# omarezz46/BayesDLL

Hardware: AMD Instinct MI355X
Metric: SG-HMC leapfrog steps/sec & HBM GB/s on ViT-L/32 params, 1/2/4/8 MI355X (higher is better)
Workload: dtype f32

## Files before the change

### bayesdll_amd/_lib.py

```python
from __future__ import annotations

import ctypes as C
import os
import threading

import numpy as np
import torch

HERE = os.path.dirname(os.path.abspath(__file__))
LIB_PATH = os.environ.get("BDL_SGMCMC_LIB", os.path.join(HERE, "libbdl_sgmcmc.so"))

BDL_OK = 0
CSGHMC, SGHMC, SGLD, SGHMC_GRAD, SGLD_GRAD, ADAM_SGHMC, ADAM_SGHMC_GRAD = range(7)
NOISE_NONE, NOISE_BUFFER, NOISE_PHILOX = 0, 1, 2
COLLECT_NONE, COLLECT_WELFORD_INIT, COLLECT_WELFORD, COLLECT_MEAN_INIT, COLLECT_MEAN = range(5)
MIX_BARE, MIX_PIPELINED, MIX_PACED = 0, 1, 2
ATTR_HEAD, ATTR_PRIOR, ATTR_SKIP, ATTR_GUNALIGNED = 0x1, 0x2, 0x4, 0x8
FLAG_FIRST_STEP, FLAG_RECIP_DIV, FLAG_MOMENTUM, FLAG_GRAD_READY = 0x1, 0x2, 0x4, 0x8
VAR_GIVEN, VAR_RAW_MOMENTS, VAR_WELFORD = 0, 1, 2
ABI_VERSION = 8

_fp = C.c_void_p


# ... 423 lines not shown
DIVERSITY_INT_MATRICES = ("disagree", "both_wrong", "kl_unbounded")
DIVERSITY_SUM_MATRICES = ("tv_sum", "kl_sum")


def diversity_totals_dtype(voters):
    P = int(voters)
    return np.dtype([(k, np.int64) for k in ("n", "n_labelled", "n_nonfinite", "voters")]
                    + [(k, np.int64, (P, P)) for k in DIVERSITY_INT_MATRICES]
                    + [(k, np.float64, (P, P)) for k in DIVERSITY_SUM_MATRICES])


class DiversityArgs(C.Structure):
    _fields_ = [("logits", _fp), ("labels", _fp), ("totals", _fp), ("workspace", _fp),
                ("batch", C.c_int64), ("voters", C.c_int32), ("classes", C.c_int32),
                ("grid_blocks", C.c_int32), ("flags", C.c_int32)]


DIVERSITY_EXPORTS = {
    "bdl_diversity_totals_bytes": (C.c_int64, [C.c_int32]),
    "bdl_diversity_workspace_bytes": (C.c_int64, [C.c_int32, C.c_int32]),
    "bdl_diversity": (C.c_int, [C.POINTER(DiversityArgs), C.c_void_p]),
}

_lib = None
_lock = threading.Lock()


def lib():
    global _lib
    if _lib is not None:
        return _lib
    with _lock:
        if _lib is None:
            if not os.path.exists(LIB_PATH):
                raise RuntimeError(
                    f"bayesdll_amd: HIP library not found at {LIB_PATH}; build it with "
                    "`make -C bayesdll_amd/csrc` (or __graft_entry__.build()). There is no CPU "
                    "fallback for the fused SG-MCMC step.")
            h = C.CDLL(LIB_PATH)
            for name, (res, argt) in (list(EXPORTS.items()) + list(DIAG_EXPORTS.items())
                                      + list(CLIP_EXPORTS.items())
                                      + list(CHAIN_STEP_EXPORTS.items())
                                      + list(STATS_EXPORTS.items())
                                      + list(ESS_EXPORTS.items())
                                      + list(LOWP_EXPORTS.items())
                                      + list(LAYERS_EXPORTS.items())
                                      + list(PREDICT_EXPORTS.items())
                                      + list(FN_EXPORTS.items())
                                      + list(TEMPER_EXPORTS.items())
                                      + list(MIXTURE_EXPORTS.items())
                                      + list(RANK_EXPORTS.items())
                                      + list(DIVERSITY_EXPORTS.items())):
                fn = getattr(h, name)
                fn.restype = res
                fn.argtypes = argt
            if h.bdl_version() != ABI_VERSION:
                raise RuntimeError(f"bayesdll_amd: ABI version mismatch ({h.bdl_version()} != "
                                   f"{ABI_VERSION}); rebuild the library")
            _lib = h
    return _lib


def check(rc: int, what: str):
    if rc != BDL_OK:
        msg = lib().bdl_last_error().decode(errors="replace")
        raise RuntimeError(f"{what} failed (status {rc}): {msg}")
    return rc


def ptr(t):
    return None if t is None else C.c_void_p(t.data_ptr())


def current_stream_handle(device=None):
    return C.c_void_p(torch.cuda.current_stream(device).cuda_stream)
# ... 9 lines not shown
```

### bayesdll_amd/csrc/bdl_api.hip

```cpp
#include <algorithm>
#include "bdl_chain_common.hpp"
#include "bdl_measure.h"

#include <mutex>
#include <vector>

namespace bdl {
namespace {

thread_local std::string g_last_error;

int g_blocks_per_cu = 2;
int g_unroll = 1;
int g_grid_stride = 1;

int device_cu_count() {
  static int cached[64] = {0};
  int dev = 0;
  if (hipGetDevice(&dev) != hipSuccess || dev < 0 || dev >= 64) return 256;
  if (cached[dev] == 0) {
    int cus = 0;
    if (hipDeviceGetAttribute(&cus, hipDeviceAttributeMultiprocessorCount, dev) != hipSuccess ||
        cus <= 0)
      cus = 256;
// ... 407 lines not shown
    return fail(BDL_ERR_RUNS, std::string(what) + ": run table exceeds 64 KiB of LDS (4096 runs, "
                "2730 with grad_base; merge parameter groups)");
  if (!s->grad && !s->grad_base)
    return fail(BDL_ERR_NULL, std::string(what) + ": grad or grad_base is required");
  if (misaligned(s->grad, 15))
    return fail(BDL_ERR_ALIGN, std::string(what) + ": grad not 16-B aligned");
  if (misaligned(s->grad_base, 7))
    return fail(BDL_ERR_ALIGN, std::string(what) + ": grad_base not 8-B aligned");
  if (s->chain_groups &&
      (s->chain_groups > 0xFFFFFFFFull ||
       (uint64_t)((s->n + 3) / 4) + s->philox_offset > 0xFFFFFFFFull))
    return fail(BDL_ERR_ARG, std::string(what) + ": stacked chains need every float4 group "
                "index below 2^32 (chain_groups, n / 4 + philox_offset)");
  if (s->noise_mode == BDL_NOISE_PHILOX)
    return check_philox_range(what, s->n, s->philox_offset, s->chain, s->chain_groups);
  return BDL_OK;
}

std::mutex g_captured_mu;
std::vector<const void*> g_captured_funcs;
thread_local hipGraphExec_t g_redirect_exec = nullptr;
thread_local hipGraphNode_t g_redirect_node = nullptr;

int launch_step(const bdl_step_args* s, const float* clip, hipStream_t stream, bool bare = false) {
  if (!s) return fail(BDL_ERR_NULL, "bdl_sgmcmc_step: null args");
  if (s->n < 0) return fail(BDL_ERR_ARG, "bdl_sgmcmc_step: n < 0");
  if (s->method < BDL_CSGHMC || s->method > BDL_SGLD_GRAD)
    return fail(BDL_ERR_ARG, "bdl_sgmcmc_step: unknown method");
  if (s->noise_mode < BDL_NOISE_NONE || s->noise_mode > BDL_NOISE_PHILOX)
    return fail(BDL_ERR_ARG, "bdl_sgmcmc_step: unknown noise mode");
  if (s->collect < BDL_COLLECT_NONE || s->collect > BDL_COLLECT_MEAN)
    return fail(BDL_ERR_ARG, "bdl_sgmcmc_step: unknown collect mode");
  if (s->n == 0) return BDL_OK;
  const bool grad_only = s->method == BDL_SGHMC_GRAD || s->method == BDL_SGLD_GRAD;
  const bool needs_mom = s->method == BDL_CSGHMC || s->method == BDL_SGHMC ||
                         s->method == BDL_SGHMC_GRAD ||
                         (s->method == BDL_SGLD && (s->flags & BDL_FLAG_MOMENTUM));
  const bool needs_prior = s->method != BDL_CSGHMC;
  if (!s->theta) return fail(BDL_ERR_NULL, "bdl_sgmcmc_step: theta is required");
  if (const int rc = check_runs_and_grad(s, "bdl_sgmcmc_step")) return rc;
  if (needs_mom && !s->mom) return fail(BDL_ERR_NULL, "bdl_sgmcmc_step: mom is required");
  if (needs_prior && !s->prior_mean)
    return fail(BDL_ERR_NULL, "bdl_sgmcmc_step: prior_mean is required for sghmc/sgld");
  if (s->noise_mode == BDL_NOISE_BUFFER && !s->noise)
    return fail(BDL_ERR_NULL, "bdl_sgmcmc_step: noise buffer is required");
  if (s->collect != BDL_COLLECT_NONE && !s->mom1)
    return fail(BDL_ERR_NULL, "bdl_sgmcmc_step: mom1 is required to collect");
// ... 10 lines not shown
  if (!k) return fail(BDL_ERR_ARG, "bdl_sgmcmc_step: unsupported method/noise/collect combination");

  const int64_t ngroups = (s->n + 3) / 4;
  const int64_t per_iter = (int64_t)kBlock * unroll;
  const int64_t cap = (int64_t)device_cu_count() * g_blocks_per_cu;
  int64_t iters = (ngroups + per_iter - 1) / per_iter;
  int64_t grid = capped_grid(iters, cap);
  int64_t iters_per_block = (iters + grid - 1) / grid;
  grid = (iters + iters_per_block - 1) / iters_per_block;

  KArgs a;
  a.theta = s->theta;
  a.grad = s->grad;
  a.mom = s->mom;
  a.prior_mean = s->prior_mean;
  a.noise = s->noise;
  a.mom1 = s->mom1;
  a.mom2 = s->mom2;
  a.runs = s->runs;
  a.gbase = s->grad_base;
  a.nruns = s->nruns;
  a.flags = s->flags;
  a.n = s->n;
  a.groups_per_block = g_grid_stride ? 0 : iters_per_block * per_iter;
  a.lr0 = s->lr[0];
  a.lr1 = s->lr[1];
  a.ns0 = s->noise_scale[0];
  a.ns1 = s->noise_scale[1];
  a.one_minus_alpha = s->one_minus_alpha;
  a.prior_sig = s->prior_sig;
  a.sigma2 = s->sigma2;
  a.n_data = s->n_data;
  a.mu = s->mu;
  a.ca = s->collect_a;
  a.cb = s->collect_b;
  a.seed = s->seed;
  a.chain = s->chain;
  a.step = s->step;
  a.clip = clip;
  a.nonfinite = s->nonfinite;
  a.goff = s->philox_offset;
  a.cgroups = (uint32_t)s->chain_groups;
  a.inv_s2 = recip_or(s->inv_sigma2, s->sigma2);
  a.inv_nd = recip_or(s->inv_n_data, s->n_data);
  a.inv_ca = recip_or(s->inv_collect_a, s->collect_a);
  a.inv_cb = recip_or(s->inv_collect_b, s->collect_b);

  if (g_redirect_exec) {
    hipGraphNodeType nt = hipGraphNodeTypeEmpty;
    hipKernelNodeParams cur{};
    if (hipGraphNodeGetType(g_redirect_node, &nt) != hipSuccess || nt != hipGraphNodeTypeKernel ||
        hipGraphKernelNodeGetParams(g_redirect_node, &cur) != hipSuccess ||
        cur.func != (void*)k) {
      (void)hipGetLastError();
      return fail(BDL_ERR_ARG, "bdl_sgmcmc_step: the redirect node is not this step's kernel");
    }
    void* kp[] = {&a};
    hipKernelNodeParams p{};
    p.func = (void*)k;
    p.gridDim = dim3((unsigned)grid);
    p.blockDim = dim3(kBlock);
    p.sharedMemBytes = (unsigned)run_lds_bytes(s);
    p.kernelParams = kp;
    const hipError_t err = hipGraphExecKernelNodeSetParams(g_redirect_exec, g_redirect_node, &p);
    if (err != hipSuccess) {
      (void)hipGetLastError();
      g_last_error = std::string("bdl_sgmcmc_step: graph node update failed: ") +
                     hipGetErrorString(err);
      return BDL_ERR_LAUNCH;
    }
// ... 191 lines not shown
  const KArgs* ka = (const KArgs*)p.kernelParams[0];
  const int64_t v[10] = {(int64_t)(uintptr_t)ka->theta, (int64_t)(uintptr_t)ka->grad,
                         (int64_t)(uintptr_t)ka->mom,   (int64_t)(uintptr_t)ka->runs,
                         (int64_t)(uintptr_t)ka->gbase, (int64_t)ka->nruns,
                         ka->n,                          (int64_t)ka->flags,
                         (int64_t)(uintptr_t)ka->mom1,  (int64_t)(uintptr_t)ka->mom2};
  for (int i = 0; i < 10; ++i) out[i] = v[i];
  return BDL_OK;
}

int bdl_graph_redirect(void* graph_exec, void* node) {
  if (graph_exec && !node) return fail(BDL_ERR_NULL, "bdl_graph_redirect: null node");
  g_redirect_exec = (hipGraphExec_t)graph_exec;
  g_redirect_node = graph_exec ? (hipGraphNode_t)node : nullptr;
  return BDL_OK;
}

const char* bdl_last_error(void) { return g_last_error.c_str(); }

int bdl_set_launch_config(int32_t blocks_per_cu, int32_t unroll, int32_t grid_stride) {
  const int prev = (g_grid_stride << 24) | (g_blocks_per_cu << 8) | g_unroll;
  g_blocks_per_cu = blocks_per_cu > 0 ? blocks_per_cu : 2;
  g_unroll = (unroll == 1 || unroll == 2 || unroll == 4) ? unroll : 1;
  g_grid_stride = grid_stride > 0 ? 1 : 0;
  return prev;
}

int bdl_build_runs(const bdl_segment* segs, int32_t nseg, int64_t n, bdl_run* out, int32_t max_runs) {
  if (!out || (nseg > 0 && !segs)) return fail(BDL_ERR_NULL, "bdl_build_runs: null pointer");
  if (n < 0 || nseg < 0 || max_runs < 1) return fail(BDL_ERR_ARG, "bdl_build_runs: bad sizes");
  int nr = 0;
  int64_t pos = 0;
  auto push = [&](int64_t end, uint32_t attr) -> bool {
    if (end <= pos) return true;
    if (nr > 0 && out[nr - 1].attr == attr) {
      out[nr - 1].end = end;
    } else {
      if (nr >= max_runs) return false;
      out[nr].end = end;
      out[nr].attr = attr;
      out[nr].pad = 0;
      ++nr;
    }
    pos = end;
    return true;
  };
  for (int i = 0; i < nseg; ++i) {
    const bdl_segment& s = segs[i];
// ... 297 lines not shown
```

### bayesdll_amd/csrc/bdl_kernels.hpp

```cpp
#pragma once
#include <hip/hip_runtime.h>

#include <stdint.h>
#include <stdio.h>
#include <string.h>

#include <algorithm>
#include <string>

#include "bdl_sgmcmc.h"

namespace bdl {

constexpr int kBlock = 256;

__device__ __forceinline__ uint4 philox4x32_10(uint4 c, uint32_t k0, uint32_t k1) {
#ifdef BDL_PHILOX_KEYS_PER_CALL
  asm volatile("" : "+s"(k0), "+s"(k1));
#endif
#if defined(BDL_PHILOX_ROUND_KEYS_PER_CALL) && !defined(BDL_PHILOX_KEYS_PER_CALL)
  asm volatile("" : "+s"(k0), "+s"(k1));
#endif
#pragma unroll
  for (int i = 0; i < 10; ++i) {
    const uint64_t p0 = (uint64_t)0xD2511F53u * c.x;
    const uint64_t p1 = (uint64_t)0xCD9E8D57u * c.z;
    const uint32_t hi0 = (uint32_t)(p0 >> 32), lo0 = (uint32_t)p0;
    const uint32_t hi1 = (uint32_t)(p1 >> 32), lo1 = (uint32_t)p1;
#ifdef BDL_PHILOX_TWO_XORS
    c = make_uint4(hi1 ^ c.y ^ k0, lo1, hi0 ^ c.w ^ k1, lo0);
#else
    c = make_uint4(__builtin_amdgcn_bitop3_b32(hi1, c.y, k0, 0x96), lo1,
                   __builtin_amdgcn_bitop3_b32(hi0, c.w, k1, 0x96), lo0);
// ... 703 lines not shown

template <int METHOD, int NOISE, int COLLECT, bool RECIP, int UNROLL>
__device__ __forceinline__ void step_variant(const KArgs& a) {
  if constexpr (COLLECT != BDL_COLLECT_NONE || !(METHOD == BDL_SGLD || METHOD == BDL_SGHMC)) {
    step_body<METHOD, NOISE, COLLECT, RECIP, UNROLL, kVarRuntime>(a);
  } else {
    if (a.flags & BDL_FLAG_GRAD_READY)
      step_body<METHOD, NOISE, COLLECT, RECIP, UNROLL, kVarGradReady>(a);
    else if (METHOD == BDL_SGLD && a.clip != nullptr)
      step_body<METHOD, NOISE, COLLECT, RECIP, UNROLL, kVarClip>(a);
    else
      step_body<METHOD, NOISE, COLLECT, RECIP, UNROLL, 0>(a);
  }
}

template <int METHOD, int NOISE, int COLLECT, int UNROLL>
__global__ __launch_bounds__(kBlock) void bdl_step_kernel(const KArgs a) {
  if (a.flags & BDL_FLAG_RECIP_DIV)
    step_variant<METHOD, NOISE, COLLECT, true, UNROLL>(a);
  else
    step_variant<METHOD, NOISE, COLLECT, false, UNROLL>(a);
}

struct AdamConst {
  bool sgd_mom, sgd_mom_read, has_m2, grad_is_mom;
  float inv_s2, inv_nd, inv_temp, inv_bc1, inv_bc2, inv_ca, inv_cb;
};

template <int NOISE, bool RECIP, bool PRIOR, bool GRADONLY, class A>
__device__ __forceinline__ void adam_core(const A& a, const AdamConst& c, float eta, float& th,
                                          float& g, float& vm, float& m, float& v, float& buf,
                                          float th0, float eps) {
  const float gs = sdiv<RECIP>(g, a.temp, c.inv_temp);
  float gU = gs;
  if constexpr (PRIOR) {
    const float d = th - th0;
    const float e = sdiv<RECIP>(d, a.sigma2, c.inv_s2);
    gU = gs + sdiv<RECIP>(e, a.n_data, c.inv_nd);
  }
  m = m * a.b1 + gU * a.omb1;
  v = v * a.b2 + (gU * gU) * a.omb2;
  const float mh = sdiv<RECIP>(m, a.bc1, c.inv_bc1);
  const float vh = sdiv<RECIP>(v, a.bc2, c.inv_bc2);
  const float den = sqrtf(vh) + a.aeps;
  const float pg = mh / den;
  const float pt = 1.0f / den;
// ... 491 lines not shown
    case BDL_COLLECT_MEAN_INIT:
      return pick_unroll<METHOD, NOISE, BDL_COLLECT_MEAN_INIT>(unroll);
    case BDL_COLLECT_MEAN:
      return pick_unroll<METHOD, NOISE, BDL_COLLECT_MEAN>(unroll);
  }
  return nullptr;
}

template <int METHOD>
StepKernel pick_noise(int noise, int collect, int unroll) {
  switch (noise) {
    case BDL_NOISE_NONE:
      return pick_collect<METHOD, BDL_NOISE_NONE>(collect, unroll);
    case BDL_NOISE_BUFFER:
      return pick_collect<METHOD, BDL_NOISE_BUFFER>(collect, unroll);
    case BDL_NOISE_PHILOX:
      return pick_collect<METHOD, BDL_NOISE_PHILOX>(collect, unroll);
  }
  return nullptr;
}

StepKernel pick_step_csghmc(int noise, int collect, int unroll);
StepKernel pick_step_csghmc_bare(int collect, int unroll);
StepKernel pick_step_sghmc(int method, int noise, int collect, int unroll);
StepKernel pick_step_sgld(int method, int noise, int collect, int unroll);
StepKernel pick_adam(int noise, int collect, bool grad_only, int unroll);

}
```

### bayesdll_amd/flat.py

```python
from __future__ import annotations

import contextlib
import ctypes as C

import numpy as np
import torch

from . import _lib as L
from .arena import default_grad_arena


def segment_attrs(names, readout_name, bias, requires_grad):
    attrs = []
    for nm, rg in zip(names, requires_grad):
        a = 0
        if readout_name is not None and readout_name in nm:
            a |= L.ATTR_HEAD
        if not ("bias" in nm and bias == "uninformative"):
            a |= L.ATTR_PRIOR
        if not rg:
            a |= L.ATTR_SKIP
        attrs.append(a)
    return attrs

# ... 358 lines not shown

    def bucket_state(self, bucket, ptrs, table=None):
        from types import SimpleNamespace
        start, end, idx = bucket
        nt = len(idx)
        if table is None:
            key = (start, tuple(ptrs))
            tab = self._grad_tables.get(key)
            if tab is None:
                dev = self.bucket_host_table(bucket, ptrs).pin_memory().to(self.device,
                                                                            non_blocking=True)
                tab = (dev[:2 * nt].view(nt, 2), nt, dev[2 * nt:])
                if len(self._grad_tables) >= 4 * GRAD_TABLE_CACHE:
                    self._grad_tables.pop(next(iter(self._grad_tables)))
                self._grad_tables[key] = tab
        else:
            if table.numel() != 3 * nt or table.dtype != torch.int64 or table.device != self.device:
                raise ValueError("bucket_state: table must be 3 x (bucket tensors) int64 on the device")
            tab = (table[:2 * nt].view(nt, 2), nt, table[2 * nt:])
        sl = (lambda v: None if v is None else v[start:end])
        return SimpleNamespace(theta=self.theta[start:end], grad=None, gbase=tab[2], runs=tab[0],
                               nruns=tab[1], mom=sl(self.mom), prior=sl(self.prior), noise=None,
                               n=end - start, device=self.device, nonfinite=self.nonfinite,
                               extra={k: v[start:end] for k, v in self.extra.items()}, timer=None)

    def grad_table(self):
        return (self.runs, self.nruns, self.gbase, self._untouched)

    def use_grad_table(self, t):
        self.runs, self.nruns, self.gbase, self._untouched = t

    def has_grad(self, i):
        if not self.requires_grad[i]:
            return False
        if self.grad_mode == "tensor":
            return i not in self._untouched
        return not self._touched or self._touched[i]

    def check_bound(self):
        vec, esz = (self.theta, 4) if self.shadow is None else (self.shadow, 2)
        for nm, p, o in zip(self.names, self.params, self.offsets):
            if p.data.data_ptr() != vec.data_ptr() + esz * o:
                raise RuntimeError(f"bayesdll_amd: parameter {nm!r} was re-allocated outside the "
                                   "sampler; rebuild the sampler state")

    def refresh_shadow(self):
        if self.shadow is not None:
# ... 74 lines not shown
```

### bayesdll_amd/kernels.py

```python
from __future__ import annotations

import ctypes as C
import os

import numpy as np
import torch

from . import _lib as L
from . import ess as E

DIV_MODE = os.environ.get("BDL_DIV_MODE", "recip")


def _div_flag(div_mode=None):
    return L.FLAG_RECIP_DIV if (div_mode or DIV_MODE) == "recip" else 0


def _inv(s):
    s = float(s)
    return 1.0 / s if s != 0.0 else 0.0


def _step_args(state, method, *, lrs, noise_scale, noise_mode, one_minus_alpha=1.0,
               prior_sig=0.0, sigma2=1.0, n_data=1.0, mu=0.0, first_step=False,
# ... 97 lines not shown
        gbs = [nb / (t * 1e-3) / 1e9 for t, (_, _, nb) in zip(ms, self.recs)]
        out = {"launches": self.count, "timed": len(ms), "avg_ms": sum(ms) / len(ms),
               "gbs": sum(gbs) / len(gbs)}
        if reset:
            self.count, self.recs = 0, []
        return out


def launch_kind(collect):
    if collect in (L.COLLECT_WELFORD, L.COLLECT_MEAN):
        return "collect"
    if collect in (L.COLLECT_WELFORD_INIT, L.COLLECT_MEAN_INIT):
        return "init"
    return "step"


def _launch(state, fn, a, adam=None, written=None):
    kind = launch_kind(a.collect)
    pend = getattr(state, "_tune_pending", None)
    if pend and written is not None and int(a.n) == int(state.n) and kind in pend and \
            not (a.flags & L.FLAG_FIRST_STEP) and \
            not torch.cuda.is_current_stream_capturing():
        _tune_kind(state, fn, kind, written)
    _use_geometry(state, kind)
    t = getattr(state, "timer", None)
    e0 = t.begin() if t is not None else None
    fn()
    if e0 is not None:
        t.end(e0, alg_bytes_per_elem(a, adam) * int(a.n))


def _written(state, method, *, grad_only, mom, extra=(), mom1=None, mom2=None):
    if grad_only:
        if getattr(state, "grad", None) is None:
            return None
        out = [state.grad]
    else:
        out = [state.theta]
    out += [t for t in (mom,) + tuple(extra) + (mom1, mom2) if t is not None]
    return out


LOWP_UNROLL = 4


def lowp_args(state, method, *, blocks=0, unroll=LOWP_UNROLL, **kw):
    if method not in (L.CSGHMC, L.SGHMC, L.SGLD):
# ... 35 lines not shown
    L.require_hip(theta, "theta")
    L.check(L.lib().bdl_lowp_shadow(theta.data_ptr(), shadow.data_ptr(), None, 0,
                                    int(theta.numel()), L.current_stream_handle(theta.device)),
            "bdl_lowp_shadow")


def sgmcmc_step(state, method, **kw):
    if getattr(state, "shadow", None) is not None:
        return lowp_step(state, method, **kw)
    a = _step_args(state, method, **kw)
    mb = kw.get("mom_buf")
    wr = _written(state, method, grad_only=method in (L.SGHMC_GRAD, L.SGLD_GRAD),
                  mom=state.mom if mb is None else mb,
                  mom1=kw.get("mom1") if kw.get("collect", L.COLLECT_NONE) else None,
                  mom2=kw.get("mom2") if kw.get("collect", L.COLLECT_NONE) else None)
    _launch(state, lambda: L.check(L.lib().bdl_sgmcmc_step(a, L.current_stream_handle(state.device)),
                                   "bdl_sgmcmc_step"), a, written=wr)


def sgmcmc_step_bare(state, **kw):
    a = _step_args(state, L.CSGHMC, **kw)
    L.check(L.lib().bdl_sgmcmc_step_bare(a, L.current_stream_handle(state.device)),
            "bdl_sgmcmc_step_bare")


def adam_step(state, method, *, adam_m, adam_v, sgd_buf=None, beta1, beta2, eps, t,
              momentum_decay, nd, temperature=1.0, grad_is_mom=False, lrs, noise_mode,
              sigma2, n_data, mu=0.0, first_step=False, momentum=False, collect=L.COLLECT_NONE,
              mom1=None, mom2=None, collect_a=1.0, collect_b=1.0, seed=0, chain=0, step=0,
              div_mode=None, noise=None, philox_offset=0):
    a = _step_args(state, method, lrs=lrs, noise_scale=(0.0, 0.0), noise_mode=noise_mode,
                   one_minus_alpha=1 - momentum_decay, sigma2=sigma2, n_data=n_data, mu=mu,
                   first_step=first_step, momentum=momentum, collect=collect, mom1=mom1,
                   mom2=mom2, collect_a=collect_a, collect_b=collect_b, seed=seed, chain=chain,
                   step=step, div_mode=div_mode, noise=noise, philox_offset=philox_offset)
    ad = L.AdamArgs()
    ad.adam_m = adam_m.data_ptr()
    ad.adam_v = adam_v.data_ptr()
    ad.sgd_buf = None if sgd_buf is None else sgd_buf.data_ptr()
    ad.beta1, ad.one_minus_beta1 = float(beta1), 1 - float(beta1)
    ad.beta2, ad.one_minus_beta2 = float(beta2), 1 - float(beta2)
    bc1, bc2 = 1 - float(beta1) ** int(t), 1 - float(beta2) ** int(t)
    ad.bias_corr1, ad.bias_corr2 = bc1, bc2
    ad.eps = float(eps)
    ad.two_alpha = 2 * float(momentum_decay)
    ad.nd = float(nd)
# ... 1250 lines not shown
        t.end(e0, alg_bytes_per_elem(a) * int(a.n1) * K_)


def philox_normal(n, seed, chain, step, device="cuda"):
    out = torch.empty(n, dtype=torch.float32, device=device)
    L.check(L.lib().bdl_philox_normal(out.data_ptr(), int(n), int(seed), int(chain), int(step),
                                      L.current_stream_handle(out.device)), "bdl_philox_normal")
    return out


_ACTIVE = [None]
LIBRARY_DEFAULT = (2, 1, 1)


def set_launch_config(blocks_per_cu=0, unroll=0, grid_stride=0):
    _ACTIVE[0] = (int(blocks_per_cu), int(unroll), int(grid_stride))
    return L.lib().bdl_set_launch_config(int(blocks_per_cu), int(unroll), int(grid_stride))


def restore_launch_config(packed):
    return set_launch_config((packed >> 8) & 0xFFFF, packed & 0xFF, (packed >> 24) & 0xFF)


def _use_geometry(state, kind="step"):
    cfg = getattr(state, {"collect": "collect_cfg", "init": "init_cfg"}.get(kind, "launch_cfg"),
                  None)
    if cfg is None:
        cfg = getattr(state, "launch_cfg", None)
    if cfg is not None and cfg != _ACTIVE[0]:
        set_launch_config(*cfg)


AUTOTUNE_CANDIDATES = ((2, 1, 1), (1, 4, 1), (3, 1, 1), (2, 4, 1), (1, 2, 1), (2, 2, 1))
AUTOTUNE_BY_METHOD = {
    "csghmc": AUTOTUNE_CANDIDATES + ((3, 4, 1), (1, 1, 1)),
    "sgld": AUTOTUNE_CANDIDATES + ((3, 4, 1), (4, 4, 1), (1, 1, 1)),
    "adam": AUTOTUNE_CANDIDATES + ((1, 1, 1), (4, 4, 1)),
}
_TUNED = {}
_TUNED_COLLECT = {}
COLLECT_EXTRA = ((1, 1, 1),)


ADAM_EXTRA = ("adam_m", "adam_v", "sgd_buf")


def _scratch_launcher(n, dev, method):
    return _scratch_launchers(n, dev, method)[0]


def _scratch_launchers(n, dev, method):
    from .flat import FlatState, moment_pair
    st = FlatState.from_segments([("w", (int(n),))], None, device=dev,
                                 need_prior=method != "csghmc",
                                 extra=ADAM_EXTRA if method == "adam" else ())
    st.theta.zero_()
    if method == "csghmc":
        kw = dict(lrs=(1e-4, 1e-4), noise_scale=(0.0, 0.0), noise_mode=L.NOISE_NONE,
# ... 95 lines not shown
def request_state_tuning(state, method):
    if os.environ.get("BDL_AUTOTUNE", "1") == "0" or int(state.n) < TUNE_ON_STATE_MIN:
        return
    state._tune_pending = {"step", "collect", "init"}
    state._tune_method = method
    state.tuned = {}


def _tune_kind(state, fn, kind, written):
    state._tune_pending.discard(kind)
    cands = tuple(AUTOTUNE_BY_METHOD.get(state._tune_method, AUTOTUNE_CANDIDATES))
    if kind != "step":
        cands += tuple(c for c in COLLECT_EXTRA if c not in cands)
    nf = getattr(state, "nonfinite", None)
    written = list(written) + ([nf] if nf is not None else [])
    need = sum(w.numel() * w.element_size() for w in written)
    free, _ = torch.cuda.mem_get_info(state.device)
    if need > TUNE_SNAPSHOT_FRACTION * free:
        state.tuned[kind] = {"skipped": f"snapshot {need >> 20} MiB > "
                                        f"{TUNE_SNAPSHOT_FRACTION:g} x free {free >> 20} MiB"}
        return
    best, times = tune_on_state(fn, written, cands, state.device)
    setattr(state, {"collect": "collect_cfg", "init": "init_cfg"}.get(kind, "launch_cfg"), best)
    state.tuned[kind] = {"best": best, "ms": {f"{c[0]}wg/cu x{c[1]}": round(t, 4)
                                              for c, t in times.items()}}


def tune_on_state(launch, written, candidates, device, reps=4):
    import numpy as np
    saved = [w.clone() for w in written]
    prev = _ACTIVE[0]
    ts = torch.cuda.current_stream(device)

    def measure(cfgs, k):
        out = {}
        for cfg in cfgs:
            set_launch_config(*cfg)
            launch()
            ev = [(torch.cuda.Event(enable_timing=True), torch.cuda.Event(enable_timing=True))
                  for _ in range(k)]
            for e0, e1 in ev:
                e0.record(ts)
                launch()
                e1.record(ts)
            torch.cuda.synchronize(device)
            out[cfg] = float(np.median([x.elapsed_time(y) for x, y in ev]))
            for w, s in zip(written, saved):
                w.copy_(s)
# ... 48 lines not shown
```

Measured before the change: 926.3.

## Add dynamic atomic work-claiming order for cSGHMC sweep and autotune it

Adds a third sweep order for the cSGHMC step. Workgroups claim fixed-size chunks through a per-stream device atomic counter pair instead of static spans or grid-stride, which is meant to even out tail imbalance across workgroups. The dynamic variants are added to the cSGHMC autotune candidates, so they are used only when the tuner picks them. Bucketed sub-states fall back to grid-stride. A drift probe kernel that records per-workgroup timestamps is also added for diagnostics. The cost is an atomic per chunk, an extra syncthreads, and a host-side claim-ring lookup plus stream-capture check on every launch.

```diff
diff --git a/bayesdll_amd/_lib.py b/bayesdll_amd/_lib.py
--- a/bayesdll_amd/_lib.py
+++ b/bayesdll_amd/_lib.py
@@ -469,6 +469,18 @@
     "bdl_diversity": (C.c_int, [C.POINTER(DiversityArgs), C.c_void_p]),
 }
 
+ORDER_SPANS, ORDER_GRID_STRIDE, ORDER_DYNAMIC = 0, 1, 2
+CLAIM_GROUPS, CLAIM_SLOTS, CLAIM_SLOTS_PER_STREAM = 2048, 16, 4
+DRIFT_EVERY, DRIFT_SAMPLES = 16, 64
+DRIFT_WORDS = 4 + 2 * DRIFT_SAMPLES
+
+ORDER_EXPORTS = {
+    "bdl_order_last": (C.c_int, [C.POINTER(C.c_int32)]),
+    "bdl_order_counters": (C.c_int, [C.c_int32, C.POINTER(C.c_uint32)]),
+    "bdl_sweep_drift": (C.c_int, [C.POINTER(StepArgs), C.c_int32, C.c_void_p, C.c_int64,
+                                  C.POINTER(C.c_int32), C.c_void_p]),
+}
+
 _lib = None
 _lock = threading.Lock()
 
@@ -497,7 +509,8 @@
                                       + list(TEMPER_EXPORTS.items())
                                       + list(MIXTURE_EXPORTS.items())
                                       + list(RANK_EXPORTS.items())
-                                      + list(DIVERSITY_EXPORTS.items())):
+                                      + list(DIVERSITY_EXPORTS.items())
+                                      + list(ORDER_EXPORTS.items())):
                 fn = getattr(h, name)
                 fn.restype = res
                 fn.argtypes = argt
diff --git a/bayesdll_amd/csrc/bdl_api.hip b/bayesdll_amd/csrc/bdl_api.hip
--- a/bayesdll_amd/csrc/bdl_api.hip
+++ b/bayesdll_amd/csrc/bdl_api.hip
@@ -1,5 +1,6 @@
 #include <algorithm>
 #include "bdl_chain_common.hpp"
+#include "bdl_claim_ring.hpp"
 #include "bdl_measure.h"
 
 #include <mutex>
@@ -453,7 +454,54 @@
 thread_local hipGraphExec_t g_redirect_exec = nullptr;
 thread_local hipGraphNode_t g_redirect_node = nullptr;
 
-int launch_step(const bdl_step_args* s, const float* clip, hipStream_t stream, bool bare = false) {
+constexpr int kClaimStride = 32;
+struct DeviceClaims {
+  uint32_t* base = nullptr;
+  ClaimRing ring{};
+};
+std::mutex g_claim_mu;
+DeviceClaims g_claims[64];
+thread_local int g_last_order = -1, g_last_slot = -1;
+
+uint32_t* claim_pair(hipStream_t stream, int* slot) {
+  bool capturing = false;
+  if (stream) {
+    hipStreamCaptureStatus cs = hipStreamCaptureStatusNone;
+    capturing = hipStreamIsCapturing(stream, &cs) != hipSuccess || cs != hipStreamCaptureStatusNone;
+    (void)hipGetLastError();
+  }
+  const bool redirect = g_redirect_exec != nullptr;
+  int dev = 0;
+  if (capturing || redirect || hipGetDevice(&dev) != hipSuccess || dev < 0 || dev >= 64)
+    return nullptr;
+  std::lock_guard<std::mutex> lk(g_claim_mu);
+  DeviceClaims& d = g_claims[dev];
+  if (!d.base) {
+    const size_t bytes = (size_t)BDL_CLAIM_SLOTS * kClaimStride * sizeof(uint32_t);
+    uint32_t* p = nullptr;
+    if (hipMalloc((void**)&p, bytes) != hipSuccess || hipMemset(p, 0, bytes) != hipSuccess ||
+        hipDeviceSynchronize() != hipSuccess) {
+      (void)hipGetLastError();
+      if (p) (void)hipFree(p);
+      return nullptr;
+    }
+    d.base = p;
+  }
+  const int sl = claim_ring_next(d.ring, (uintptr_t)stream, capturing, redirect);
+  if (sl < 0) return nullptr;
+  *slot = sl;
+  return d.base + (size_t)sl * kClaimStride;
+}
+
+struct DriftReq {
+  int order;
+  uint64_t* records;
+  int64_t record_bytes;
+  int32_t* grid;
+};
+
+int launch_step(const bdl_step_args* s, const float* clip, hipStream_t stream, bool bare = false,
+                const DriftReq* drift = nullptr) {
   if (!s) return fail(BDL_ERR_NULL, "bdl_sgmcmc_step: null args");
   if (s->n < 0) return fail(BDL_ERR_ARG, "bdl_sgmcmc_step: n < 0");
   if (s->method < BDL_CSGHMC || s->method > BDL_SGLD_GRAD)
@@ -510,7 +558,8 @@
   a.nruns = s->nruns;
   a.flags = s->flags;
   a.n = s->n;
-  a.groups_per_block = g_grid_stride ? 0 : iters_per_block * per_iter;
+  const int order = drift ? drift->order : g_grid_stride;
+  a.groups_per_block = order ? 0 : iters_per_block * per_iter;
   a.lr0 = s->lr[0];
   a.lr1 = s->lr[1];
   a.ns0 = s->noise_scale[0];
@@ -534,6 +583,31 @@
   a.inv_ca = recip_or(s->inv_collect_a, s->collect_a);
   a.inv_cb = recip_or(s->inv_collect_b, s->collect_b);
 
+  int slot = -1;
+  uint32_t* pair = nullptr;
+  if (order == 2 && s->method == BDL_CSGHMC &&
+      run_lds_bytes(s) + 16 <= (size_t)kMaxRuns * sizeof(bdl_run))
+    pair = claim_pair(stream, &slot);
+  g_last_order = pair ? 2 : (order ? 1 : 0);
+  g_last_slot = slot;
+  const int32_t citers = (int32_t)(BDL_CLAIM_GROUPS / per_iter);
+  if (pair) grid = capped_grid((iters + citers - 1) / citers, cap);
+  if (drift) {
+    if (order == 2 && !pair)
+      return fail(BDL_ERR_ARG, "bdl_sweep_drift: no counter pair for the dynamic order here");
+    if (drift->record_bytes < grid * (int64_t)(BDL_DRIFT_WORDS * sizeof(uint64_t)))
+      return fail(BDL_ERR_ARG, "bdl_sweep_drift: records too small for the launch's workgroups");
+    *drift->grid = (int32_t)grid;
+    hipLaunchKernelGGL(pick_drift(unroll, pair != nullptr), dim3((unsigned)grid), dim3(kBlock),
+                       run_lds_bytes(s), stream, a, pair, citers, drift->records);
+    return launched("bdl_sweep_drift");
+  }
+  if (pair) {
+    hipLaunchKernelGGL(pick_step_csghmc_dyn(s->noise_mode, s->collect, unroll, bare),
+                       dim3((unsigned)grid), dim3(kBlock), run_lds_bytes(s), stream, a, pair, citers);
+    return launched("bdl_sgmcmc_step");
+  }
+
   if (g_redirect_exec) {
     hipGraphNodeType nt = hipGraphNodeTypeEmpty;
     hipKernelNodeParams cur{};
@@ -771,8 +845,54 @@
   const int prev = (g_grid_stride << 24) | (g_blocks_per_cu << 8) | g_unroll;
   g_blocks_per_cu = blocks_per_cu > 0 ? blocks_per_cu : 2;
   g_unroll = (unroll == 1 || unroll == 2 || unroll == 4) ? unroll : 1;
-  g_grid_stride = grid_stride > 0 ? 1 : 0;
+  g_grid_stride = grid_stride == 2 ? 2 : (grid_stride > 0 ? 1 : 0);
   return prev;
+}
+
+int bdl_order_last(int32_t* slot) {
+  if (slot) *slot = g_last_slot;
+  return g_last_order;
+}
+
+int bdl_order_counters(int32_t device, uint32_t* out) {
+  if (!out) return fail(BDL_ERR_NULL, "bdl_order_counters: null out");
+  if (device < 0 || device >= 64) return fail(BDL_ERR_ARG, "bdl_order_counters: bad device");
+  std::fill(out, out + 2 * BDL_CLAIM_SLOTS, 0u);
+  std::lock_guard<std::mutex> lk(g_claim_mu);
+  const uint32_t* base = g_claims[device].base;
+  if (!base) return BDL_OK;
+  int cur = 0;
+  uint32_t host[BDL_CLAIM_SLOTS * kClaimStride];
+  if (hipGetDevice(&cur) != hipSuccess || hipSetDevice(device) != hipSuccess) {
+    (void)hipGetLastError();
+    return fail(BDL_ERR_LAUNCH, "bdl_order_counters: cannot select the device");
+  }
+  const bool ok = hipDeviceSynchronize() == hipSuccess &&
+                  hipMemcpy(host, base, sizeof(host), hipMemcpyDeviceToHost) == hipSuccess;
+  (void)hipSetDevice(cur);
+  if (!ok) {
+    (void)hipGetLastError();
+    return fail(BDL_ERR_LAUNCH, "bdl_order_counters: reading the counters failed");
+  }
+  for (int i = 0; i < BDL_CLAIM_SLOTS; ++i) {
+    out[2 * i] = host[i * kClaimStride];
+    out[2 * i + 1] = host[i * kClaimStride + 1];
+  }
+  return BDL_OK;
+}
+
+int bdl_sweep_drift(const bdl_step_args* s, int32_t order, uint64_t* records, int64_t record_bytes,
+                    int32_t* grid, void* stream) {
+  if (const int rc = no_redirect("bdl_sweep_drift")) return rc;
+  if (!s || !records || !grid) return fail(BDL_ERR_NULL, "bdl_sweep_drift: null argument");
+  if (s->method != BDL_CSGHMC || s->noise_mode != BDL_NOISE_NONE || s->collect != BDL_COLLECT_NONE)
+    return fail(BDL_ERR_ARG, "bdl_sweep_drift: the probe runs the cSGHMC explore sweep only "
+                "(no noise, no collect)");
+  if (order < 0 || order > 2) return fail(BDL_ERR_ARG, "bdl_sweep_drift: order must be 0, 1 or 2");
+  if (misaligned(records, 7)) return fail(BDL_ERR_ALIGN, "bdl_sweep_drift: records not 8-B aligned");
+  if (s->n == 0) return fail(BDL_ERR_ARG, "bdl_sweep_drift: n == 0");
+  const DriftReq req{order, records, record_bytes, grid};
+  return launch_step(s, nullptr, (hipStream_t)stream, false, &req);
 }
 
 int bdl_build_runs(const bdl_segment* segs, int32_t nseg, int64_t n, bdl_run* out, int32_t max_runs) {
diff --git a/bayesdll_amd/csrc/bdl_claim_ring.hpp b/bayesdll_amd/csrc/bdl_claim_ring.hpp
--- /dev/null
+++ b/bayesdll_amd/csrc/bdl_claim_ring.hpp
@@ -0,0 +1,29 @@
+#pragma once
+#include <stdint.h>
+
+#include "bdl_order.h"
+
+namespace bdl {
+
+struct ClaimRing {
+  uintptr_t owner[BDL_CLAIM_SLOTS];
+  bool bound[BDL_CLAIM_SLOTS];
+  int cursor;
+};
+
+inline int claim_ring_next(ClaimRing& ring, uintptr_t stream, bool capturing, bool redirect) {
+  if (capturing || redirect) return -1;
+  int owned = 0;
+  for (int i = 0; i < BDL_CLAIM_SLOTS; ++i) owned += ring.bound[i] && ring.owner[i] == stream;
+  for (int k = 0; k < BDL_CLAIM_SLOTS; ++k) {
+    const int s = (ring.cursor + k) % BDL_CLAIM_SLOTS;
+    if (ring.bound[s] ? ring.owner[s] != stream : owned >= BDL_CLAIM_SLOTS_PER_STREAM) continue;
+    ring.bound[s] = true;
+    ring.owner[s] = stream;
+    ring.cursor = (s + 1) % BDL_CLAIM_SLOTS;
+    return s;
+  }
+  return -1;
+}
+
+}
diff --git a/bayesdll_amd/csrc/bdl_kernels.hpp b/bayesdll_amd/csrc/bdl_kernels.hpp
--- a/bayesdll_amd/csrc/bdl_kernels.hpp
+++ b/bayesdll_amd/csrc/bdl_kernels.hpp
@@ -9,6 +9,7 @@
 #include <string>
 
 #include "bdl_sgmcmc.h"
+#include "bdl_order.h"
 
 namespace bdl {
 
@@ -758,6 +759,155 @@
     step_variant<METHOD, NOISE, COLLECT, false, UNROLL>(a);
 }
 
+struct NoProbe {
+  __device__ __forceinline__ void begin() {}
+  __device__ __forceinline__ void tick(int64_t) {}
+  __device__ __forceinline__ void end() {}
+};
+
+struct DriftProbe {
+  uint64_t* __restrict__ rec;
+  uint32_t it;
+  __device__ __forceinline__ void begin() {
+    if (threadIdx.x == 0) rec[0] = wall_clock64();
+  }
+  __device__ __forceinline__ void tick(int64_t iter) {
+    if (it % BDL_DRIFT_EVERY == 0) {
+      const uint32_t s = it / BDL_DRIFT_EVERY;
+      if (s < BDL_DRIFT_SAMPLES && threadIdx.x == 0) {
+        rec[4 + 2 * s] = wall_clock64();
+        rec[5 + 2 * s] = (uint64_t)iter;
+      }
+    }
+    ++it;
+  }
+  __device__ __forceinline__ void end() {
+    __threadfence();
+    __syncthreads();
+    if (threadIdx.x == 0) {
+      rec[1] = wall_clock64();
+      rec[2] = min((it + BDL_DRIFT_EVERY - 1) / BDL_DRIFT_EVERY, (uint32_t)BDL_DRIFT_SAMPLES);
+      rec[3] = it;
+    }
+  }
+};
+
+template <int METHOD, int NOISE, int COLLECT, bool RECIP, int UNROLL, bool DYN, class PROBE>
+__device__ __forceinline__ void csg_sweep(const KArgs& a, uint32_t* __restrict__ claim,
+                                          int32_t citers, PROBE probe) {
+  static_assert(is_csghmc_sweep<METHOD>(), "the dynamic order exists for the cSGHMC sweeps");
+  __shared__ uint32_t s_claim[2];
+  const StepConst c = make_step_const<METHOD, COLLECT, kVarRuntime>(a);
+  const int64_t ngroups = (a.n + 3) >> 2;
+  const int64_t nfull = a.n >> 2;
+  constexpr int64_t kIter = (int64_t)kBlock * UNROLL;
+  const int64_t cgroups = (int64_t)citers * kIter;
+  int64_t g0, g1, gstep;
+  if constexpr (DYN) {
+    g0 = (int64_t)blockIdx.x * cgroups;
+    g1 = min(g0 + cgroups, ngroups);
+    gstep = kIter;
+  } else if (a.groups_per_block > 0) {
+    g0 = (int64_t)blockIdx.x * a.groups_per_block;
+    g1 = min(g0 + a.groups_per_block, ngroups);
+    gstep = kIter;
+  } else {
+    g0 = (int64_t)blockIdx.x * kIter;
+    g1 = ngroups;
+    gstep = (int64_t)gridDim.x * kIter;
+  }
+  stage_runs(a);
+  probe.begin();
+  uint32_t bad = 0, nxt = 0;
+  int r = -1, par = 0;
+  while (g0 < g1) {
+    if constexpr (DYN) {
+      if (threadIdx.x == 0) nxt = gridDim.x + atomicAdd(claim, 1u);
+    }
+    if (r < 0) r = find_run_lds(a.nruns, g0 * 4);
+    if constexpr (COLLECT != BDL_COLLECT_NONE && !csg_collect_per_run<COLLECT, UNROLL>()) {
+      for (int64_t gb = g0; gb < g1; gb += gstep) {
+        while (r < a.nruns - 1 && run_end(r) <= gb * 4) ++r;
+        const int64_t gend = min(gb + kIter, g1);
+        const uint32_t attr = run_attr(r);
+        const bool full = gend == gb + kIter && gend <= nfull;
+        if (full && run_end(r) >= gend * 4 && !(attr & kNoFastPath))
+          chunk_fast_dispatch<METHOD, NOISE, COLLECT, RECIP, UNROLL>(a, c, gb, attr,
+                                                                      run_grad(a, r), bad);
+        else if (full && multi_run_ok(a.nruns, r, gend * 4))
+          chunk_multi<METHOD, NOISE, COLLECT, RECIP, UNROLL>(a, c, gb, r, bad);
+        else
+          chunk_slow<METHOD, NOISE, COLLECT, RECIP, UNROLL>(a, c, gb, gend, r, bad);
+        probe.tick(gb / kIter);
+      }
+    } else {
+      for (int64_t gb = g0; gb < g1;) {
+        while (r < a.nruns - 1 && run_end(r) <= gb * 4) ++r;
+        const uint32_t attr = run_attr(r);
+        const int64_t lim = min(min(run_end(r) >> 2, nfull), g1);
+        if (!(attr & kNoFastPath) && gb + kIter <= lim) {
+          const bool head = (attr & BDL_ATTR_HEAD) != 0;
+          const float eta = head ? a.lr1 : a.lr0, ns = head ? a.ns1 : a.ns0;
+          float* gp = run_grad(a, r);
+          do {
+            chunk_fast<METHOD, NOISE, COLLECT, RECIP, UNROLL, false, false>(a, c, gb, eta, ns, gp,
+                                                                            bad);
+            probe.tick(gb / kIter);
+            gb += gstep;
+          } while (gb + kIter <= lim);
+          continue;
+        }
+        const int64_t gend = min(gb + kIter, g1);
+        if (gend == gb + kIter && gend <= nfull && multi_run_ok(a.nruns, r, gend * 4))
+          chunk_multi<METHOD, NOISE, COLLECT, RECIP, UNROLL>(a, c, gb, r, bad);
+        else
+          chunk_slow<METHOD, NOISE, COLLECT, RECIP, UNROLL>(a, c, gb, gend, r, bad);
+        probe.tick(gb / kIter);
+        gb += gstep;
+      }
+    }
+    if constexpr (!DYN) {
+      break;
+    } else {
+      if (threadIdx.x == 0) s_claim[par] = nxt;
+      __syncthreads();
+      const uint32_t blk = s_claim[par];
+      par ^= 1;
+      g0 = (int64_t)blk * cgroups;
+      g1 = min(g0 + cgroups, ngroups);
+    }
+  }
+  report_nonfinite(a, bad);
+  probe.end();
+  if constexpr (DYN) {
+    if (threadIdx.x == 0 && atomicAdd(claim + 1, 1u) == gridDim.x - 1) {
+      __hip_atomic_store(claim, 0u, __ATOMIC_RELAXED, __HIP_MEMORY_SCOPE_AGENT);
+      __hip_atomic_store(claim + 1, 0u, __ATOMIC_RELAXED, __HIP_MEMORY_SCOPE_AGENT);
+    }
+  }
+}
+
+template <int METHOD, int NOISE, int COLLECT, int UNROLL>
+__global__ __launch_bounds__(kBlock) void bdl_step_dyn_kernel(const KArgs a, uint32_t* claim,
+                                                              int32_t citers) {
+  if (a.flags & BDL_FLAG_RECIP_DIV)
+    csg_sweep<METHOD, NOISE, COLLECT, true, UNROLL, true, NoProbe>(a, claim, citers, NoProbe{});
+  else
+    csg_sweep<METHOD, NOISE, COLLECT, false, UNROLL, true, NoProbe>(a, claim, citers, NoProbe{});
+}
+
+template <int UNROLL, bool DYN>
+__global__ __launch_bounds__(kBlock) void bdl_drift_kernel(const KArgs a, uint32_t* claim,
+                                                           int32_t citers, uint64_t* rec) {
+  DriftProbe p{rec + (size_t)blockIdx.x * BDL_DRIFT_WORDS, 0};
+  if (a.flags & BDL_FLAG_RECIP_DIV)
+    csg_sweep<BDL_CSGHMC, BDL_NOISE_NONE, BDL_COLLECT_NONE, true, UNROLL, DYN, DriftProbe>(
+        a, claim, citers, p);
+  else
+    csg_sweep<BDL_CSGHMC, BDL_NOISE_NONE, BDL_COLLECT_NONE, false, UNROLL, DYN, DriftProbe>(
+        a, claim, citers, p);
+}
+
 struct AdamConst {
   bool sgd_mom, sgd_mom_read, has_m2, grad_is_mom;
   float inv_s2, inv_nd, inv_temp, inv_bc1, inv_bc2, inv_ca, inv_cb;
@@ -1295,6 +1445,10 @@
 
 StepKernel pick_step_csghmc(int noise, int collect, int unroll);
 StepKernel pick_step_csghmc_bare(int collect, int unroll);
+using DynKernel = void (*)(const KArgs, uint32_t*, int32_t);
+using DriftKernel = void (*)(const KArgs, uint32_t*, int32_t, uint64_t*);
+DynKernel pick_step_csghmc_dyn(int noise, int collect, int unroll, bool bare);
+DriftKernel pick_drift(int unroll, bool dyn);
 StepKernel pick_step_sghmc(int method, int noise, int collect, int unroll);
 StepKernel pick_step_sgld(int method, int noise, int collect, int unroll);
 StepKernel pick_adam(int noise, int collect, bool grad_only, int unroll);
diff --git a/bayesdll_amd/csrc/bdl_step_csghmc_dyn.hip b/bayesdll_amd/csrc/bdl_step_csghmc_dyn.hip
--- /dev/null
+++ b/bayesdll_amd/csrc/bdl_step_csghmc_dyn.hip
@@ -0,0 +1,61 @@
+#include "bdl_kernels.hpp"
+
+namespace bdl {
+namespace {
+
+template <int METHOD, int NOISE, int COLLECT>
+DynKernel dyn_unroll(int unroll) {
+  switch (unroll) {
+    case 1:
+      return bdl_step_dyn_kernel<METHOD, NOISE, COLLECT, 1>;
+    case 4:
+      return bdl_step_dyn_kernel<METHOD, NOISE, COLLECT, 4>;
+    default:
+      return bdl_step_dyn_kernel<METHOD, NOISE, COLLECT, 2>;
+  }
+}
+
+template <int METHOD, int NOISE>
+DynKernel dyn_collect(int collect, int unroll) {
+  switch (collect) {
+    case BDL_COLLECT_NONE:
+      return dyn_unroll<METHOD, NOISE, BDL_COLLECT_NONE>(unroll);
+    case BDL_COLLECT_WELFORD_INIT:
+      return dyn_unroll<METHOD, NOISE, BDL_COLLECT_WELFORD_INIT>(unroll);
+    case BDL_COLLECT_WELFORD:
+      return dyn_unroll<METHOD, NOISE, BDL_COLLECT_WELFORD>(unroll);
+    case BDL_COLLECT_MEAN_INIT:
+      return dyn_unroll<METHOD, NOISE, BDL_COLLECT_MEAN_INIT>(unroll);
+    case BDL_COLLECT_MEAN:
+      return dyn_unroll<METHOD, NOISE, BDL_COLLECT_MEAN>(unroll);
+  }
+  return nullptr;
+}
+
+}
+
+DynKernel pick_step_csghmc_dyn(int noise, int collect, int unroll, bool bare) {
+  if (bare) return dyn_collect<kMethodBare, BDL_NOISE_NONE>(collect, unroll);
+  switch (noise) {
+    case BDL_NOISE_NONE:
+      return dyn_collect<BDL_CSGHMC, BDL_NOISE_NONE>(collect, unroll);
+    case BDL_NOISE_BUFFER:
+      return dyn_collect<BDL_CSGHMC, BDL_NOISE_BUFFER>(collect, unroll);
+    case BDL_NOISE_PHILOX:
+      return dyn_collect<BDL_CSGHMC, BDL_NOISE_PHILOX>(collect, unroll);
+  }
+  return nullptr;
+}
+
+DriftKernel pick_drift(int unroll, bool dyn) {
+  switch (unroll) {
+    case 1:
+      return dyn ? bdl_drift_kernel<1, true> : bdl_drift_kernel<1, false>;
+    case 4:
+      return dyn ? bdl_drift_kernel<4, true> : bdl_drift_kernel<4, false>;
+    default:
+      return dyn ? bdl_drift_kernel<2, true> : bdl_drift_kernel<2, false>;
+  }
+}
+
+}
diff --git a/bayesdll_amd/flat.py b/bayesdll_amd/flat.py
--- a/bayesdll_amd/flat.py
+++ b/bayesdll_amd/flat.py
@@ -404,7 +404,8 @@
         return SimpleNamespace(theta=self.theta[start:end], grad=None, gbase=tab[2], runs=tab[0],
                                nruns=tab[1], mom=sl(self.mom), prior=sl(self.prior), noise=None,
                                n=end - start, device=self.device, nonfinite=self.nonfinite,
-                               extra={k: v[start:end] for k, v in self.extra.items()}, timer=None)
+                               extra={k: v[start:end] for k, v in self.extra.items()}, timer=None,
+                               bucket=True)
 
     def grad_table(self):
         return (self.runs, self.nruns, self.gbase, self._untouched)
diff --git a/bayesdll_amd/kernels.py b/bayesdll_amd/kernels.py
--- a/bayesdll_amd/kernels.py
+++ b/bayesdll_amd/kernels.py
@@ -143,7 +143,7 @@
             not (a.flags & L.FLAG_FIRST_STEP) and \
             not torch.cuda.is_current_stream_capturing():
         _tune_kind(state, fn, kind, written)
-    _use_geometry(state, kind)
+    _use_geometry(state, kind, sub=getattr(state, "bucket", False))
     t = getattr(state, "timer", None)
     e0 = t.begin() if t is not None else None
     fn()
@@ -225,6 +225,57 @@
     a = _step_args(state, L.CSGHMC, **kw)
     L.check(L.lib().bdl_sgmcmc_step_bare(a, L.current_stream_handle(state.device)),
             "bdl_sgmcmc_step_bare")
+
+
+def last_order():
+    slot = C.c_int32(-1)
+    return int(L.lib().bdl_order_last(C.byref(slot))), int(slot.value)
+
+
+def order_counters(device=None):
+    dev = _device(device)
+    out = (C.c_uint32 * (2 * L.CLAIM_SLOTS))()
+    L.check(L.lib().bdl_order_counters(int(dev.index or 0), out), "bdl_order_counters")
+    return np.ctypeslib.as_array(out).reshape(L.CLAIM_SLOTS, 2).copy()
+
+
+def sweep_drift(state, order, **kw):
+    a = _step_args(state, L.CSGHMC, noise_mode=L.NOISE_NONE, **kw)
+    cap = 16 * 1024
+    rec = torch.zeros(cap, L.DRIFT_WORDS, dtype=torch.int64, device=state.device)
+    grid = C.c_int32(0)
+    L.check(L.lib().bdl_sweep_drift(a, int(order), rec.data_ptr(),
+                                    rec.numel() * rec.element_size(), C.byref(grid),
+                                    L.current_stream_handle(state.device)), "bdl_sweep_drift")
+    torch.cuda.synchronize(state.device)
+    return rec[:grid.value].cpu()
+
+
+def drift_summary(rec, fractions=(0.125, 0.25, 0.375, 0.5, 0.625, 0.75, 0.875)):
+    rec = rec.numpy().astype(np.int64)
+    t0, t1, ns = rec[:, 0], rec[:, 1], rec[:, 2]
+    start, end = int(t0.min()), int(t1.max())
+    span = end - start
+    grid = rec.shape[0]
+    out = {"workgroups": int(grid), "span_ticks": int(span),
+           "iterations": int(rec[:, 3].sum()),
+           "iterations_min_max": [int(rec[:, 3].min()), int(rec[:, 3].max())],
+           "tail_loss": float(1.0 - (t1 - t0).sum() / (grid * span)),
+           "ramp_loss": float((t0 - start).sum() / (grid * span)),
+           "end_loss": float((end - t1).sum() / (grid * span)),
+           "truncated": bool((rec[:, 3] > L.DRIFT_EVERY * L.DRIFT_SAMPLES).any()),
+           "spread": []}
+    ts, it = rec[:, 4::2], rec[:, 5::2]
+    valid = np.arange(L.DRIFT_SAMPLES)[None, :] < ns[:, None]
+    for f in fractions:
+        T = start + f * span
+        seen = valid & (ts <= T)
+        have = seen.any(axis=1)
+        last = np.where(seen, it, -1).max(axis=1)[have]
+        sp = int(last.max() - last.min()) if last.size else 0
+        out["spread"].append({"at": f, "iterations": sp, "rows": round(sp / grid, 2),
+                              "workgroups_sampled": int(have.sum())})
+    return out
 
 
 def adam_step(state, method, *, adam_m, adam_v, sgd_buf=None, beta1, beta2, eps, t,
@@ -1521,18 +1572,24 @@
     return set_launch_config((packed >> 8) & 0xFFFF, packed & 0xFF, (packed >> 24) & 0xFF)
 
 
-def _use_geometry(state, kind="step"):
+def _use_geometry(state, kind="step", sub=False):
     cfg = getattr(state, {"collect": "collect_cfg", "init": "init_cfg"}.get(kind, "launch_cfg"),
                   None)
     if cfg is None:
         cfg = getattr(state, "launch_cfg", None)
+    if sub:
+        act = cfg or _ACTIVE[0]
+        if act is not None and act[2] == L.ORDER_DYNAMIC:
+            cfg = (act[0], act[1], L.ORDER_GRID_STRIDE)
     if cfg is not None and cfg != _ACTIVE[0]:
         set_launch_config(*cfg)
 
 
 AUTOTUNE_CANDIDATES = ((2, 1, 1), (1, 4, 1), (3, 1, 1), (2, 4, 1), (1, 2, 1), (2, 2, 1))
 AUTOTUNE_BY_METHOD = {
-    "csghmc": AUTOTUNE_CANDIDATES + ((3, 4, 1), (1, 1, 1)),
+    "csghmc": (AUTOTUNE_CANDIDATES + ((3, 4, 1), (1, 1, 1))
+               + tuple((b, u, L.ORDER_DYNAMIC)
+                       for b, u, _ in AUTOTUNE_CANDIDATES + ((3, 4, 1), (1, 1, 1)))),
     "sgld": AUTOTUNE_CANDIDATES + ((3, 4, 1), (4, 4, 1), (1, 1, 1)),
     "adam": AUTOTUNE_CANDIDATES + ((1, 1, 1), (4, 4, 1)),
 }
@@ -1674,8 +1731,10 @@
         return
     best, times = tune_on_state(fn, written, cands, state.device)
     setattr(state, {"collect": "collect_cfg", "init": "init_cfg"}.get(kind, "launch_cfg"), best)
-    state.tuned[kind] = {"best": best, "ms": {f"{c[0]}wg/cu x{c[1]}": round(t, 4)
-                                              for c, t in times.items()}}
+    state.tuned[kind] = {"best": best,
+                         "ms": {f"{c[0]}wg/cu x{c[1]}" + (" dynamic" if c[2] == L.ORDER_DYNAMIC
+                                                          else ""): round(t, 4)
+                                for c, t in times.items()}}
 
 
 def tune_on_state(launch, written, candidates, device, reps=4):
diff --git a/include/bdl_order.h b/include/bdl_order.h
--- /dev/null
+++ b/include/bdl_order.h
@@ -0,0 +1,31 @@
+#ifndef BDL_ORDER_H
+#define BDL_ORDER_H
+
+#include <stdint.h>
+
+#include "bdl_sgmcmc.h"
+
+#define BDL_CLAIM_GROUPS 2048
+#define BDL_CLAIM_SLOTS 16
+#define BDL_CLAIM_SLOTS_PER_STREAM 4
+
+#define BDL_DRIFT_EVERY 16
+#define BDL_DRIFT_SAMPLES 64
+#define BDL_DRIFT_WORDS (4 + 2 * BDL_DRIFT_SAMPLES)
+
+#ifdef __cplusplus
+extern "C" {
+#endif
+
+int bdl_order_last(int32_t* slot);
+
+int bdl_order_counters(int32_t device, uint32_t* out);
+
+int bdl_sweep_drift(const bdl_step_args* args, int32_t order, uint64_t* records,
+                    int64_t record_bytes, int32_t* grid, void* hip_stream);
+
+#ifdef __cplusplus
+}
+#endif
+
+#endif
```

Result: faster. 1007 (median of 6 runs) (+8.7%).
